# hku-mars/FAST_LIO

Measured on NVIDIA H100. Metric: scans/sec (30k-pt scan, 1M-pt map iEKF), higher is better.
Workload: dtype f32 geometry / f64 filter

## Files before the change

fast_lio_b200/csrc/filter.cu:

```cuda
#include <dlfcn.h>

#include <algorithm>
#include <chrono>
#include <cstdlib>

#include <cub/device/device_select.cuh>

#include "filter.h"
#include "gj.cuh"

namespace fl {

constexpr int PSTRIDE = 96;
constexpr size_t P2P_MAIL_BYTES = sizeof(unsigned long long) * 2 * 2 * P2P_MAX_RANKS * PSTRIDE;
constexpr int SEARCH_THREADS = 256;
constexpr int SEARCH_C_THREADS = 256;
constexpr int RESID_THREADS = 256;
constexpr int MAX_LOGS = 16;

__device__ __forceinline__ void pdl_wait() { asm volatile("griddepcontrol.wait;" ::: "memory"); }
__device__ __forceinline__ void pdl_launch() { asm volatile("griddepcontrol.launch_dependents;" ::: "memory"); }

__device__ __forceinline__ int tri12(int a, int b) { return a * 12 - (a * (a - 1)) / 2 + (b - a); }

// ... 960 lines not shown

__global__ void k_flags_clear(unsigned char* __restrict__ flag_add, unsigned char* __restrict__ flag_no, const int* __restrict__ n, int n_max) {
    const int q = blockIdx.x * blockDim.x + threadIdx.x;
    if (q < n_max && q >= *n) { flag_add[q] = 0; flag_no[q] = 0; }
}

struct NcclUniqueId { char internal[128]; };
struct NcclApi {
    void* lib = nullptr;
    int (*GetUniqueId)(NcclUniqueId*) = nullptr;
    int (*CommInitRank)(void**, int, NcclUniqueId, int) = nullptr;
    int (*AllReduce)(const void*, void*, size_t, int, int, void*, cudaStream_t) = nullptr;
    int (*CommDestroy)(void*) = nullptr;
    const char* (*GetErrorString)(int) = nullptr;
};
static NcclApi* load_nccl() {
    static NcclApi api;
    if (api.lib) return &api;
    const char* names[] = {"libnccl.so.2", "libnccl.so"};
    for (const char* nm : names) { api.lib = dlopen(nm, RTLD_NOW | RTLD_GLOBAL); if (api.lib) break; }
    if (!api.lib) { set_last_error("NCCL: cannot dlopen libnccl.so.2: %s", dlerror()); return nullptr; }
    api.GetUniqueId = (int (*)(NcclUniqueId*))dlsym(api.lib, "ncclGetUniqueId");
    api.CommInitRank = (int (*)(void**, int, NcclUniqueId, int))dlsym(api.lib, "ncclCommInitRank");
    api.AllReduce = (int (*)(const void*, void*, size_t, int, int, void*, cudaStream_t))dlsym(api.lib, "ncclAllReduce");
    api.CommDestroy = (int (*)(void*))dlsym(api.lib, "ncclCommDestroy");
    api.GetErrorString = (const char* (*)(int))dlsym(api.lib, "ncclGetErrorString");
    if (!api.GetUniqueId || !api.CommInitRank || !api.AllReduce || !api.CommDestroy) {
        set_last_error("NCCL: missing symbols in libnccl");
        api.lib = nullptr;
        return nullptr;
    }
    return &api;
}
int nccl_unique_id(void* out128) {
    NcclApi* api = load_nccl();
    if (!api) return FL_ERR_NCCL;
    NcclUniqueId id;
    int rc = api->GetUniqueId(&id);
    if (rc != 0) { set_last_error("ncclGetUniqueId failed: %d", rc); return FL_ERR_NCCL; }
    memcpy(out128, &id, 128);
    return FL_OK;
}

Filter::Filter(Map* map, int max_points) : map_(map), max_points_(max_points) {
    memset(&scan_, 0, sizeof(scan_));
    for (int i = 0; i < NDOF; i++) limit_[i] = 0.001;
}
Filter::~Filter() {
    cudaSetDevice(map_->device());
    if (comm_ && nccl_) nccl_->CommDestroy(comm_);
    for (int r = 0; r < P2P_MAX_RANKS; r++) if (peer_ptr_[r]) cudaIpcCloseMemHandle(peer_ptr_[r]);
    mailbox_.release(); p2p_.release();
    body_.release(); nearest_.release(); nearest_cnt_.release(); selected_.release(); normvec_.release(); plane_.release(); srange_.release();
    partials_.release(); red_.release(); ctl_.release(); ctl0_.release(); logs_.release(); pub_.release();
    mi_world_.release(); mi_flag_add_.release(); mi_flag_no_.release(); mi_list_add_.release(); mi_list_no_.release(); mi_tmp_.release(); mi_counts_.release();
    d_bind_.release();
    if (h_ctl_) cudaFreeHost(h_ctl_);
    if (ev0_) cudaEventDestroy(ev0_);
    if (ev1_) cudaEventDestroy(ev1_);
}

int Filter::init() {
    FL_CUDA(cudaSetDevice(map_->device()));
    if (const char* e = getenv("FASTLIO_B200_NO_PDL")) pdl_ = !(e[0] == '1');
    if (const char* e = getenv("FASTLIO_B200_NO_MIRROR")) mirror_ = !(e[0] == '1');
    if (const char* e = getenv("FASTLIO_B200_SEARCH")) search_mode_ = atoi(e) ? 1 : 0;
    FL_CHECK(ctl_.reserve(sizeof(FilterCtl)));
    FL_CHECK(ctl0_.reserve(sizeof(FilterCtl)));
    FL_CHECK(red_.reserve(sizeof(double) * PSTRIDE));
    FL_CHECK(logs_.reserve(sizeof(PassLog) * MAX_LOGS));
    FL_CHECK(pub_.reserve(512));
    FL_CUDA(cudaMemsetAsync(pub_.ptr, 0, 512, stream()));
    FL_CUDA(cudaMallocHost(&h_ctl_, sizeof(FilterCtl)));
    memset(h_ctl_, 0, sizeof(FilterCtl));
    FL_CUDA(cudaMemsetAsync(ctl_.ptr, 0, sizeof(FilterCtl), stream()));
    FL_CUDA(cudaMemsetAsync(ctl0_.ptr, 0, sizeof(FilterCtl), stream()));
    FL_CUDA(cudaMemsetAsync(logs_.ptr, 0, sizeof(PassLog) * MAX_LOGS, stream()));
    int dev = map_->device(), occ = 0;
    FL_CUDA(cudaDeviceGetAttribute(&sms_, cudaDevAttrMultiProcessorCount, dev));
    if (const char* e = getenv("FASTLIO_B200_SEARCH_OCC")) search_occ_ = atoi(e);
    if (search_occ_ == 6) FL_CUDA(cudaOccupancyMaxActiveBlocksPerMultiprocessor(&occ, k_search<6>, SEARCH_THREADS, 0));
    else if (search_occ_ == 5) FL_CUDA(cudaOccupancyMaxActiveBlocksPerMultiprocessor(&occ, k_search<5>, SEARCH_THREADS, 0));
    else FL_CUDA(cudaOccupancyMaxActiveBlocksPerMultiprocessor(&occ, k_search<4>, SEARCH_THREADS, 0));
    search_grid_max_ = sms_ * std::max(1, occ);
    if (const char* e = getenv("FASTLIO_B200_LEGACY")) fused_ = !(e[0] == '1');
    FL_CUDA(cudaOccupancyMaxActiveBlocksPerMultiprocessor(&occ, k_update<false, 1>, UPD_THREADS, 0));
    upd_capacity_[0][0] = sms_ * std::max(1, occ);
    FL_CUDA(cudaOccupancyMaxActiveBlocksPerMultiprocessor(&occ, k_update<true, 1>, UPD_THREADS, 0));
    upd_capacity_[1][0] = sms_ * std::max(1, occ);
    FL_CUDA(cudaOccupancyMaxActiveBlocksPerMultiprocessor(&occ, k_update<false, 2>, 2 * UPD_THREADS, 0));
    upd_capacity_[0][1] = sms_ * occ;
    FL_CUDA(cudaOccupancyMaxActiveBlocksPerMultiprocessor(&occ, k_update<true, 2>, 2 * UPD_THREADS, 0));
    upd_capacity_[1][1] = sms_ * occ;
    FL_CUDA(cudaOccupancyMaxActiveBlocksPerMultiprocessor(&occ, k_update_n<false, 1>, UPD_THREADS, 0));
    upd_n_capacity_[0][0] = std::min(upd_capacity_[0][0], sms_ * std::max(1, occ));
    FL_CUDA(cudaOccupancyMaxActiveBlocksPerMultiprocessor(&occ, k_update_n<true, 1>, UPD_THREADS, 0));
    upd_n_capacity_[1][0] = std::min(upd_capacity_[1][0], sms_ * std::max(1, occ));
    FL_CUDA(cudaOccupancyMaxActiveBlocksPerMultiprocessor(&occ, k_update_n<false, 2>, 2 * UPD_THREADS, 0));
    upd_n_capacity_[0][1] = std::min(upd_capacity_[0][1], sms_ * occ);
    FL_CUDA(cudaOccupancyMaxActiveBlocksPerMultiprocessor(&occ, k_update_n<true, 2>, 2 * UPD_THREADS, 0));
    upd_n_capacity_[1][1] = std::min(upd_capacity_[1][1], sms_ * occ);
    FL_CHECK(d_bind_.reserve(2 * sizeof(int)));
    FL_CUDA(cudaMemsetAsync(d_bind_.ptr, 0, 2 * sizeof(int), stream()));
    FL_CHECK(partials_.reserve(sizeof(double) * PSTRIDE * (size_t)std::max(upd_capacity_[0][0], upd_capacity_[1][0])));
    max_resid_grid_ = sms_;
    FL_CHECK(partials_.reserve(sizeof(double) * PSTRIDE * (size_t)max_resid_grid_));
    FL_CHECK(reserve(std::max(1, max_points_)));
    return FL_OK;
}

int Filter::reserve(int nq) {
    FL_CHECK(body_.reserve(sizeof(float4) * (size_t)nq));
    FL_CHECK(nearest_.reserve(sizeof(float4) * KNN_K * (size_t)nq));
    { const size_t had = nearest_cnt_.bytes; FL_CHECK(nearest_cnt_.reserve(sizeof(int) * (size_t)nq)); if (nearest_cnt_.bytes != had) FL_CUDA(cudaMemsetAsync(nearest_cnt_.ptr, 0, nearest_cnt_.bytes, stream())); }
    FL_CHECK(selected_.reserve((size_t)nq));
    FL_CHECK(normvec_.reserve(sizeof(float4) * (size_t)nq));
    scan_.nearest = nearest_.as<float4>();
    scan_.nearest_cnt = nearest_cnt_.as<int>();
    scan_.selected = selected_.as<unsigned char>();
    scan_.normvec = normvec_.as<float4>();
    FL_CHECK(plane_.reserve(sizeof(float4) * (size_t)nq));
    scan_.plane = plane_.as<float4>();
    FL_CHECK(srange_.reserve(sizeof(double) * (size_t)nq));
    scan_.srange = srange_.as<double>();
    FL_CHECK(mi_world_.reserve(sizeof(float4) * (size_t)nq));
    FL_CHECK(mi_flag_add_.reserve((size_t)nq));
    FL_CHECK(mi_flag_no_.reserve((size_t)nq));
    FL_CHECK(mi_list_add_.reserve(sizeof(float4) * (size_t)nq));
    FL_CHECK(mi_list_no_.reserve(sizeof(float4) * (size_t)nq));
    FL_CHECK(mi_counts_.reserve(sizeof(int) * 2));
    size_t tmp = 0;
    FL_CUDA(cub::DeviceSelect::Flagged(nullptr, tmp, (const float4*)nullptr, (const unsigned char*)nullptr, (float4*)nullptr, (int*)nullptr, nq));
    FL_CHECK(mi_tmp_.reserve(tmp));
    return FL_OK;
}

int Filter::set_params(int max_iter, const double* limit23, int extrinsic_est_en) {
    if (max_iter < 1 || max_iter + 1 > MAX_LOGS) { set_last_error("set_params: max_iter must be in [1, %d]", MAX_LOGS - 1); return FL_ERR_ARG; }
    max_iter_ = max_iter;
    if (limit23) for (int i = 0; i < NDOF; i++) limit_[i] = limit23[i];
    extrinsic_est_ = extrinsic_est_en ? 1 : 0;
    return FL_OK;
}

int Filter::set_scan_device(const float4* d_body, int nq) {
    FL_CHECK(bind_scan(d_body, nq));
    if (stream_bound_) FL_CUDA(cudaMemsetAsync(d_bind_.as<int>() + 1, 0, sizeof(int), stream()));
    return FL_OK;
}
int Filter::bind_scan(const float4* d_body, int nq) {
    if (nq < 0) { set_last_error("scan: nq < 0"); return FL_ERR_ARG; }
    FL_CUDA(cudaSetDevice(map_->device()));
    FL_CHECK(reserve(std::max(1, nq)));
    scan_.body = d_body;
    scan_.Q = nq;
    if (!shard_set_) { scan_.q_begin = 0; scan_.q_end = nq; }
    dev_count_ = false;
    return FL_OK;
// ... 87 lines not shown
        if (nranks_ > 1 && !p2p_on_) {
            for (int pass = 0; pass <= max_iter_; pass++) {
                FL_CHECK(launch_update(1, 1, 0));
                int rc = nccl_->AllReduce(red_.ptr, red_.ptr, NRED,  8,  0, comm_, st);
                if (rc != 0) { set_last_error("ncclAllReduce failed: %d", rc); return FL_ERR_NCCL; }
                FL_CHECK(launch_update(1, 3, 0));
                launches_ += 2;
            }
        } else {
            FL_CHECK(launch_update(max_iter_ + 1, nranks_ > 1 ? 2 : 0, 0));
            launches_ = 1;
        }
        FL_CUDA(cudaGetLastError());
        return FL_OK;
    }
    for (int pass = 0; pass <= max_iter_; pass++) {
        FL_CHECK(launch_search_only());
        FL_CHECK(launch_residual_only());
        launches_ += 2;
        if (nranks_ > 1 && !p2p_on_) {
            cudaStream_t st = stream();
            int rc = nccl_->AllReduce(red_.ptr, red_.ptr, NRED,  8,  0, comm_, st);
            if (rc != 0) { set_last_error("ncclAllReduce failed: %d", rc); return FL_ERR_NCCL; }
            FilterCtl* c = ctl_.as<FilterCtl>(); double* rg = red_.as<double>(); PassLog* lg = logs_.as<PassLog>();
            if (extrinsic_est_) { if (solver_) k_solve_only<true, 1><<<1, RESID_THREADS, 0, st>>>(c, rg, scan_, lg); else k_solve_only<true, 0><<<1, RESID_THREADS, 0, st>>>(c, rg, scan_, lg); }
            else { if (solver_) k_solve_only<false, 1><<<1, RESID_THREADS, 0, st>>>(c, rg, scan_, lg); else k_solve_only<false, 0><<<1, RESID_THREADS, 0, st>>>(c, rg, scan_, lg); }
            launches_++;
        }
    }
    FL_CUDA(cudaGetLastError());
    return FL_OK;
}

UpdArgs Filter::upd_args(int max_passes, int mode, int search_only) {
    UpdArgs a;
    a.m = map_->view();
    if (search_mode_ == 0) a.m.dir.cap = 0;
    a.sc = scan_; a.ctl = ctl_.as<FilterCtl>(); a.partials = partials_.as<double>(); a.red_g = red_.as<double>();
    a.logs = logs_.as<PassLog>(); a.p2p = p2p_.as<P2PState>();
    a.mode = mode; a.max_passes = max_passes; a.search_only = search_only;
    a.pub = pub_.as<unsigned long long>(); a.nonce = ++launch_nonce_;
    { const char* e = getenv("FASTLIO_B200_DBG"); a.dbg = e ? atoi(e) : 0; }
    a.pose_from_search = 0;
    return a;
}

int Filter::launch_update(int max_passes, int mode, int search_only, cudaStream_t st) {
    FL_CUDA(cudaSetDevice(map_->device()));
    const int nq = scan_.q_end - scan_.q_begin;
    const UpdArgs a = upd_args(max_passes, mode, search_only);
    const int cap = upd_capacity_[extrinsic_est_ ? 1 : 0][0];
    int workers = mode == 3 ? 0 : std::min(cap - 1, (nq + UPD_THREADS - 1) / UPD_THREADS);
    if (workers < 0) workers = 0;
    FL_CUDA(launch_upd(workers, pdl_, a, upd_pair(nq), st));
    return FL_OK;
}

int Filter::upd_pair(int nq) const {
    if (const char* e = getenv("FASTLIO_B200_PAIR")) if (e[0] == '1') return 1;
    const int tiles = (nq + UPD_THREADS - 1) / UPD_THREADS;
    return tiles >= 1 && tiles <= upd_capacity_[extrinsic_est_ ? 1 : 0][1] - 1 ? 2 : 1;
}
cudaError_t Filter::launch_upd(int workers, bool pdl, const UpdArgs& a, int pair, cudaStream_t st) {
    const int block = pair * UPD_THREADS;
    if (extrinsic_est_) return pair == 2 ? launch_pdl(k_update<true, 2>, workers + 1, block, st, pdl, a)
                                         : launch_pdl(k_update<true, 1>, workers + 1, block, st, pdl, a);
    return pair == 2 ? launch_pdl(k_update<false, 2>, workers + 1, block, st, pdl, a)
                     : launch_pdl(k_update<false, 1>, workers + 1, block, st, pdl, a);
}

int Filter::launch_search_only() {
    FL_CUDA(cudaSetDevice(map_->device()));
    const int nq = scan_.q_end - scan_.q_begin;
    if (fused()) return launch_update(1, 0, 1);
    if (search_mode_ == 1) {
        const int cgrid = std::max(1, (nq + SEARCH_C_THREADS - 1) / SEARCH_C_THREADS);
        FL_CUDA(launch_pdl(k_search_c, cgrid, SEARCH_C_THREADS, stream(), pdl_, map_->view(), scan_, (const FilterCtl*)ctl_.as<FilterCtl>()));
        return FL_OK;
    }
    const int sgrid = std::max(1, std::min(search_grid_max_, (nq * 32 + SEARCH_THREADS - 1) / SEARCH_THREADS));
    const FilterCtl* cc = ctl_.as<FilterCtl>();
    if (search_occ_ == 6) FL_CUDA(launch_pdl(k_search<6>, sgrid, SEARCH_THREADS, stream(), pdl_, map_->view(), scan_, cc));
    else if (search_occ_ == 5) FL_CUDA(launch_pdl(k_search<5>, sgrid, SEARCH_THREADS, stream(), pdl_, map_->view(), scan_, cc));
    else FL_CUDA(launch_pdl(k_search<4>, sgrid, SEARCH_THREADS, stream(), pdl_, map_->view(), scan_, cc));
    return FL_OK;
}
int Filter::launch_residual_only() {
    FL_CUDA(cudaSetDevice(map_->device()));
    const int nq = scan_.q_end - scan_.q_begin;
    resid_grid_ = std::min(max_resid_grid_ - 1, (nq + RESID_THREADS - 1) / RESID_THREADS) + 1;
    const int mode = nranks_ > 1 ? (p2p_on_ ? 2 : 1) : 0;
    P2PState* p2p = p2p_.as<P2PState>();
    FilterCtl* c = ctl_.as<FilterCtl>(); double* pp = partials_.as<double>(); double* rg = red_.as<double>(); PassLog* lg = logs_.as<PassLog>();
    cudaStream_t st = stream();
    if (extrinsic_est_) {
        if (solver_) FL_CUDA(launch_pdl(k_residual<true, 1>, resid_grid_, RESID_THREADS, st, pdl_, scan_, c, pp, rg, mode, lg, p2p));
        else FL_CUDA(launch_pdl(k_residual<true, 0>, resid_grid_, RESID_THREADS, st, pdl_, scan_, c, pp, rg, mode, lg, p2p));
    } else {
        if (solver_) FL_CUDA(launch_pdl(k_residual<false, 1>, resid_grid_, RESID_THREADS, st, pdl_, scan_, c, pp, rg, mode, lg, p2p));
        else FL_CUDA(launch_pdl(k_residual<false, 0>, resid_grid_, RESID_THREADS, st, pdl_, scan_, c, pp, rg, mode, lg, p2p));
    }
    FL_CUDA(cudaGetLastError());
    return FL_OK;
}
int Filter::sync() {
    FL_CUDA(cudaSetDevice(map_->device()));
    FL_CUDA(cudaStreamSynchronize(stream()));
    return FL_OK;
}

int Filter::download_state(double* x26, double* P, int* n_pass) {
    FL_CUDA(cudaSetDevice(map_->device()));
    FL_CUDA(cudaStreamSynchronize(stream()));
    if (!(mirror_ && h_ctl_->done)) {
        FL_CUDA(cudaMemcpyAsync(h_ctl_, ctl_.ptr, offsetof(FilterCtl, P_prop), cudaMemcpyDeviceToHost, stream()));
        FL_CUDA(cudaStreamSynchronize(stream()));
    }
// ... 383 lines not shown
```

fast_lio_b200/csrc/filter.h:

```cpp
#pragma once
#include "lie.cuh"
#include "map.h"

namespace fl {

struct PassLog {
    int searched, valid, effct, converged;
    double res_sum;
    double HtH[144];
    double Hth[12];
    double x_after[XLEN];
};

struct FilterCtl {
    int iter;
    int t;
    int converge;
    int done;
    int n_pass;
    int max_iter;
    int extrinsic_est;
    int error;
    int ticket;
    int gen;
// ... 54 lines not shown
    int launch_residual_only();
    int download_state(double* x26, double* P, int* n_pass);
    int sync();
    int update_on_stream(const float* d_body, int nq, double* d_x26, double* d_P, double R, int* d_status2, cudaStream_t st);
    int get_nearest_on_stream(float* d_pts, int* d_cnt, int nq, cudaStream_t st);
    int get_selected_on_stream(unsigned char* d_out, int nq, cudaStream_t st);
    int update_scan_on_stream(const float4* d_body, const int* d_n, int n_max, double* d_x26, double* d_P, double R, int* d_status2, cudaStream_t st);
    int capacity() const;

    int map_incremental(double filter_size_map_min, int ekf_inited, int* n_to_add, int* n_no_downsample, int* added);
    int map_incremental_on_stream(double filter_size_map_min, int ekf_inited, int* d_out4, cudaStream_t st);
    int get_nearest(float* out_pts, int* out_cnt, int nq);
    int complete_neighbours();
    int get_selected(unsigned char* out, int nq);
    int get_pass_logs(PassLog* out, int cap, int* n);
    int comm_init(int nranks, int rank, const void* nccl_unique_id_128);
    int set_shard(int q_begin, int q_end);
    int p2p_local_handle(void* out64);
    int p2p_connect(int nranks, int rank, const void* handles64);
    int p2p_barrier();

    void set_fused(bool on) { fused_ = on; }
    bool fused() const { return fused_ && solver_ == 1; }
    int gpu_launches() const { return launches_; }
    const long long* host_ns() const { return host_ns_; }
    const float4* nearest_device() const { return scan_.nearest; }
    const ScanView& scan() const { return scan_; }
    cudaStream_t stream() const { return map_->stream(); }
    Map* map() const { return map_; }
    const FilterCtl* ctl_device() const { return ctl_.as<FilterCtl>(); }

private:
    int reserve(int nq);
    int update_any(const float* body_xyzi, const float4* d_body, int nq, double* x26, double* P, double R, double* solve_time_s);
    Map* map_;
    int max_points_;
    int max_iter_ = 4;
    double limit_[NDOF];
    int extrinsic_est_ = 0;
    int solver_ = 1;
    bool mirror_ = true;
    bool pdl_ = true;
    int search_occ_ = 5;
    int search_mode_ = 1;
    ScanView scan_;
    DeviceBuffer srange_;
    DeviceBuffer body_, nearest_, nearest_cnt_, selected_, normvec_, plane_, partials_, red_, ctl_, ctl0_, logs_;
    DeviceBuffer mi_world_, mi_flag_add_, mi_flag_no_, mi_list_add_, mi_list_no_, mi_tmp_, mi_counts_;
    FilterCtl* h_ctl_ = nullptr;
    cudaEvent_t ev0_ = nullptr, ev1_ = nullptr;
    int sms_ = 0, search_grid_max_ = 0, max_resid_grid_ = 0, resid_grid_ = 1;
    bool fused_ = true;
    DeviceBuffer pub_;
    unsigned launch_nonce_ = 0;
    int upd_capacity_[2][2] = {{0, 0}, {0, 0}};
    int launch_update(int max_passes, int mode, int search_only) { return launch_update(max_passes, mode, search_only, stream()); }
    int launch_update(int max_passes, int mode, int search_only, cudaStream_t st);
    int upd_pair(int nq) const;
    cudaError_t launch_upd(int workers, bool pdl, const UpdArgs& a, int pair) { return launch_upd(workers, pdl, a, pair, stream()); }
    cudaError_t launch_upd(int workers, bool pdl, const UpdArgs& a, int pair, cudaStream_t st);
    int device_form_scope(const char* what, bool update) const;
    UpdArgs upd_args(int max_passes, int mode, int search_only);
    int bind_scan(const float4* d_body, int nq);
    bool dev_count_ = false;
    int q_max_ = 0;
    const float4* scan_body_ = nullptr;
    bool stream_bound_ = false;
    DeviceBuffer d_bind_;
    int upd_n_capacity_[2][2] = {{0, 0}, {0, 0}};
    int read_binding();
    int launches_ = 0;
    long long host_ns_[4] = {0, 0, 0, 0};
    bool shard_set_ = false;
    bool neighbours_complete_ = true;
    NcclApi* nccl_ = nullptr;
    void* comm_ = nullptr;
    int nranks_ = 1, rank_ = 0;
    DeviceBuffer mailbox_, p2p_;
    void* peer_ptr_[P2P_MAX_RANKS] = {nullptr};
    bool p2p_on_ = false;
};

}
```

fast_lio_b200/csrc/update.cuh:

```cuda
#pragma once

namespace fl {

constexpr int UPD_THREADS = 256;
constexpr int UPD_WARPS = UPD_THREADS / 32;

struct UpdArgs {
    MapView m;
    ScanView sc;
    FilterCtl* ctl;
    double* partials;
    double* red_g;
    PassLog* logs;
    P2PState* p2p;
    unsigned long long* pub;
    unsigned nonce;
    int mode;
    int max_passes;
    int search_only;
    int dbg;
    int pose_from_search;
};

struct SolverSm {
    double Pp[NDOF * NDOF];
    double Pt[NDOF * NDOF];
    double W1[NDOF * NDOF];
    double Y[12 * NDOF];
    double Wm[12 * 13];
    double HTH[144];
    double wred[UPD_WARPS][PSTRIDE];
    double red[PSTRIDE];
    double x[XLEN], xprop[XLEN], xnew[XLEN];
    double dx[NDOF], dxn[NDOF], dxu[NDOF], limit[NDOF];
    double J[2][9], M2[4];
    double Bprop[6];
    double R;
    int iter, t, converge, done, n_pass, max_iter, error;
    int effct, ok, finish, searched, late;
    int row_k[12];
};
template <bool EXTR> struct WorkerSm {
    static constexpr int STAGE = 32 * RowStage<EXTR>::RS + 96;
    double stage[UPD_WARPS][STAGE];
    double wred[UPD_WARPS][PSTRIDE];
    WalkPool walks;
    unsigned pose_bits[28];
    unsigned flags;
    int abort;
};

__device__ __forceinline__ int ld_acquire(const int* p) {
    int v;
    asm volatile("ld.acquire.gpu.global.s32 %0, [%1];" : "=r"(v) : "l"(p) : "memory");
    return v;
}
__device__ __forceinline__ void st_release(int* p, int v) { asm volatile("st.release.gpu.global.s32 [%0], %1;" ::"l"(p), "r"(v) : "memory"); }
constexpr long long SPIN_LIMIT = 3000000000ll;

constexpr int PUB_WORDS = 29;
__device__ __forceinline__ unsigned pub_tag(unsigned nonce, int pass) { return (nonce << 8) | (unsigned)(pass & 0xff); }
__device__ __forceinline__ void pub_store(unsigned long long* p, unsigned tag, unsigned payload) {
    asm volatile("st.relaxed.gpu.global.u64 [%0], %1;" ::"l"(p), "l"(((unsigned long long)tag << 32) | payload) : "memory");
}
__device__ __forceinline__ unsigned long long pub_load(const unsigned long long* p) {
    unsigned long long v;
    asm volatile("ld.relaxed.gpu.global.u64 %0, [%1];" : "=l"(v) : "l"(p) : "memory");
    return v;
}
__device__ __forceinline__ void pub_publish(unsigned long long* pub, unsigned tag, const double* x, int converge, int done, int lane) {
    if (lane < 28) {
        const unsigned long long bits = (unsigned long long)__double_as_longlong(x[lane >> 1]);
        pub_store(pub + lane, tag, (lane & 1) ? (unsigned)(bits >> 32) : (unsigned)bits);
    } else if (lane == 28) {
        pub_store(pub + 28, tag, (converge ? 1u : 0u) | (done ? 2u : 0u));
    }
}


__device__ __forceinline__ void cell_scan_chunks(const MapView& m, int start, int cnt, int c0, int c1, float qx, float qy, float qz, TBest& kb) {
    const int4* list = reinterpret_cast<const int4*>(m.dir.lists + start);
    int4 ia = make_int4(0, 0, 0, 0), ib = make_int4(0, 0, 0, 0);
    if (c0 < c1) {
        ia = __ldg(&list[2 * c0]);
        if (cnt - 8 * c0 > 4) ib = __ldg(&list[2 * c0 + 1]);
    }
#pragma unroll 1
    for (int c = c0; c < c1; c++) {
        const int n8 = cnt - 8 * c;
        float4 p0, p1, p2, p3, p4, p5, p6, p7;
        p1 = p2 = p3 = p4 = p5 = p6 = p7 = make_float4(0.f, 0.f, 0.f, 0.f);
        p0 = __ldg(&m.pts[ia.x]);
        if (n8 > 1) p1 = __ldg(&m.pts[ia.y]);
        if (n8 > 2) p2 = __ldg(&m.pts[ia.z]);
        if (n8 > 3) p3 = __ldg(&m.pts[ia.w]);
        if (n8 > 4) p4 = __ldg(&m.pts[ib.x]);
        if (n8 > 5) p5 = __ldg(&m.pts[ib.y]);
        if (n8 > 6) p6 = __ldg(&m.pts[ib.z]);
        if (n8 > 7) p7 = __ldg(&m.pts[ib.w]);
        int4 na = ia, nb = ib;
        if (c + 1 < c1) {
            na = __ldg(&list[2 * c + 2]);
            if (n8 > 12) nb = __ldg(&list[2 * c + 3]);
        }
        cell_consider(p0, ia.x, qx, qy, qz, kb);
        cell_consider(p1, ia.y, qx, qy, qz, kb);
        cell_consider(p2, ia.z, qx, qy, qz, kb);
        cell_consider(p3, ia.w, qx, qy, qz, kb);
        cell_consider(p4, ib.x, qx, qy, qz, kb);
        cell_consider(p5, ib.y, qx, qy, qz, kb);
        cell_consider(p6, ib.z, qx, qy, qz, kb);
        cell_consider(p7, ib.w, qx, qy, qz, kb);
        ia = na; ib = nb;
    }
}

struct PairXch {
    float d[KNN_K][32];
    int idx[KNN_K][32];
};

__device__ __forceinline__ void pair_merge(const PairXch& X, int lane, TBest& kb) {
// ... 178 lines not shown
#pragma unroll 1
            for (int i = 0; i < 9; i++) S.J[warp][i] = J.m[i];
            const D3 seg = mul33v(J, l);
            S.dx[idx] = l.x; S.dx[idx + 1] = l.y; S.dx[idx + 2] = l.z;
            S.dxn[idx] = seg.x; S.dxn[idx + 1] = seg.y; S.dxn[idx + 2] = seg.z;
        } else if (warp == 2) {
            double d0, d1;
            S2_boxminus_B(ld3(S.x + X_GRAV), ld3(S.xprop + X_GRAV), S.Bprop, d0, d1);
            S2_congruence_B(ld3(S.x + X_GRAV), ld3(S.xprop + X_GRAV), S.Bprop, d0, d1, S.M2);
            S.dx[21] = d0; S.dx[22] = d1;
            S.dxn[21] = S.M2[0] * d0 + S.M2[1] * d1;
            S.dxn[22] = S.M2[2] * d0 + S.M2[3] * d1;
        }
    }
    if (warp == 3 && lane < 15) {
        const int b = lane / 3, c = lane % 3;
        const int dof = b == 0 ? 0 : 9 + 3 * (b - 1);
        const int xo = b == 0 ? X_POS : (b == 1 ? X_OFFT : (b == 2 ? X_VEL : (b == 3 ? X_BG : X_BA)));
        const double d = S.x[xo + c] - S.xprop[xo + c];
        S.dx[dof + c] = d; S.dxn[dof + c] = d;
    }
    sol_sync();
#pragma unroll 1
    for (int e = tid; e < n * n; e += UPD_THREADS) {
        const int i = e / n, j = e - i * n;
        const double* row = &S.Pp[i * n];
        double v;
        if (j >= 3 && j < 9) {
            const int b = j >= 6, base = 3 + 3 * b, r = j - base;
            v = S.J[b][3 * r] * row[base] + S.J[b][3 * r + 1] * row[base + 1] + S.J[b][3 * r + 2] * row[base + 2];
        } else if (j >= 21) {
            const int r = j - 21;
            v = S.M2[2 * r] * row[21] + S.M2[2 * r + 1] * row[22];
        } else v = row[j];
        S.W1[e] = v;
    }
    sol_sync();
#pragma unroll 1
    for (int e = tid; e < n * n; e += UPD_THREADS) {
        const int i = e / n, j = e - i * n;
        double v;
        if (i >= 3 && i < 9) {
            const int b = i >= 6, base = 3 + 3 * b, r = i - base;
            v = S.J[b][3 * r] * S.W1[base * n + j] + S.J[b][3 * r + 1] * S.W1[(base + 1) * n + j] + S.J[b][3 * r + 2] * S.W1[(base + 2) * n + j];
        } else if (i >= 21) {
            const int r = i - 21;
            v = S.M2[2 * r] * S.W1[21 * n + j] + S.M2[2 * r + 1] * S.W1[22 * n + j];
        } else v = S.W1[e];
        S.Pt[e] = v;
    }
    sol_sync();
}

__device__ void sol_reduce(SolverSm& S, const double* __restrict__ partials, int nwork) {
    const int tid = threadIdx.x, lane = tid & 31, warp = tid >> 5;
    double a0 = 0.0, a1 = 0.0, a2 = 0.0;
    for (int b = warp; b < nwork; b += 8 * UPD_WARPS) {
        double v[8][3];
#pragma unroll
        for (int k = 0; k < 8; k++) {
            const int bb = b + k * UPD_WARPS;
            const double* row = partials + (size_t)bb * PSTRIDE;
            v[k][0] = v[k][1] = v[k][2] = 0.0;
            if (bb < nwork) { v[k][0] = __ldcg(&row[lane]); v[k][1] = __ldcg(&row[lane + 32]); v[k][2] = __ldcg(&row[lane + 64]); }
        }
#pragma unroll
        for (int k = 0; k < 8; k++) { a0 += v[k][0]; a1 += v[k][1]; a2 += v[k][2]; }
    }
    S.wred[warp][lane] = a0; S.wred[warp][lane + 32] = a1; S.wred[warp][lane + 64] = a2;
    sol_sync();
    if (tid < PSTRIDE) {
        double v = 0.0;
#pragma unroll
        for (int w = 0; w < UPD_WARPS; w++) v += S.wred[w][tid];
        S.red[tid] = v;
        if (tid < 78) {
            int a = 0, rem = tid;
            while (rem >= 12 - a) { rem -= 12 - a; a++; }
            const int b = a + rem;
            S.HTH[a * 12 + b] = v; S.HTH[b * 12 + a] = v;
        }
    }
    sol_sync();
}
__device__ void sol_expand(SolverSm& S) {
    const int tid = threadIdx.x;
    if (tid < 144) { const int a = tid / 12, b = tid - a * 12; S.HTH[tid] = S.red[a <= b ? tri12(a, b) : tri12(b, a)]; }
    sol_sync();
}

__device__ void sol_exchange(SolverSm& S, P2PState* p2p) {
    const int nr = p2p->nranks, me = p2p->rank;
    const unsigned long long epoch = p2p->epoch + 1;
    const unsigned long long tag = (epoch & 0xffffffffull) << 32;
    const int par = (int)(epoch & 1ull);
    for (int idx = threadIdx.x; idx < nr * PSTRIDE; idx += UPD_THREADS) {
        const int r = idx / PSTRIDE, o = idx - r * PSTRIDE;
        const unsigned long long bits = (unsigned long long)__double_as_longlong(S.red[o]);
        unsigned long long* dst = reinterpret_cast<unsigned long long*>(p2p->peer_mail[r]) + (((size_t)par * nr + me) * PSTRIDE + o) * 2;
        asm volatile("st.volatile.global.u64 [%0], %1;" ::"l"(dst), "l"(tag | (bits & 0xffffffffull)) : "memory");
        asm volatile("st.volatile.global.u64 [%0], %1;" ::"l"(dst + 1), "l"(tag | (bits >> 32)) : "memory");
    }
    sol_sync();
    if (threadIdx.x < PSTRIDE) {
        const unsigned long long* mail = reinterpret_cast<const unsigned long long*>(p2p->peer_mail[me]) + (size_t)par * nr * PSTRIDE * 2;
        double v = 0.0;
        bool late = false;
        for (int r = 0; r < nr && !late; r++) {
            const unsigned long long* src = mail + ((size_t)r * PSTRIDE + threadIdx.x) * 2;
            unsigned long long lo = 0, hi = 0;
            const long long t0 = clock64();
            while (true) {
                asm volatile("ld.volatile.global.u64 %0, [%1];" : "=l"(lo) : "l"(src) : "memory");
                asm volatile("ld.volatile.global.u64 %0, [%1];" : "=l"(hi) : "l"(src + 1) : "memory");
                if ((lo & 0xffffffff00000000ull) == tag && (hi & 0xffffffff00000000ull) == tag) break;
                if (clock64() - t0 > SPIN_LIMIT) { late = true; break; }
            }
            v += __longlong_as_double((long long)((hi << 32) | (lo & 0xffffffffull)));
        }
        S.red[threadIdx.x] = v;
// ... 122 lines not shown
        }
        asm volatile("bar.sync 1, 128;" ::: "memory");
#pragma unroll 1
        for (int e = t4; e < n * n; e += 128) {
            const int i = e / n, j = e - i * n;
            double v = 0.0;
#pragma unroll
            for (int a = 0; a < NE; a++) v = fma(S.Pt[i * n + a] * Rinv, S.Y[a * n + j], v);
            S.W1[e] = S.Pt[e] - v;
        }
    }
    sol_sync();
    if (tid < XLEN) { ctl->x[tid] = S.xnew[tid]; if (lg) lg->x_after[tid] = S.xnew[tid]; }
    if (tid == 32) { ctl->t = S.t; ctl->converge = S.converge; ctl->iter = S.iter + 1; ctl->n_pass = S.n_pass + 1; ctl->done = finish; }
    if (!finish) {
#pragma unroll 1
        for (int e = tid; e < n * n; e += UPD_THREADS) ctl->P[e] = S.Pt[e];
    } else {
#pragma unroll 1
        for (int e = tid; e < n * n; e += UPD_THREADS) {
            const int i = e / n, j = e - i * n;
            double v;
            if (i >= 3 && i < 9) {
                const int b = i >= 6, base = 3 + 3 * b, r = i - base;
                v = S.J[b][3 * r] * S.W1[base * n + j] + S.J[b][3 * r + 1] * S.W1[(base + 1) * n + j] + S.J[b][3 * r + 2] * S.W1[(base + 2) * n + j];
            } else if (i >= 21) {
                const int r = i - 21;
                v = S.M2[2 * r] * S.W1[21 * n + j] + S.M2[2 * r + 1] * S.W1[22 * n + j];
            } else v = S.W1[e];
            S.Pt[e] = v;
        }
        sol_sync();
#pragma unroll 1
        for (int e = tid; e < n * n; e += UPD_THREADS) {
            const int i = e / n, j = e - i * n;
            const double* row = &S.Pt[i * n];
            double v;
            if (j >= 3 && j < 9) {
                const int b = j >= 6, base = 3 + 3 * b, r = j - base;
                v = S.J[b][3 * r] * row[base] + S.J[b][3 * r + 1] * row[base + 1] + S.J[b][3 * r + 2] * row[base + 2];
            } else if (j >= 21) {
                const int r = j - 21;
                v = S.M2[2 * r] * row[21] + S.M2[2 * r + 1] * row[22];
            } else v = row[j];
            ctl->P[e] = v;
        }
    }
    sol_sync();
    if (tid < XLEN) S.x[tid] = S.xnew[tid];
    if (tid == 32) { S.iter++; S.n_pass++; S.done = finish; }
    sol_sync();
}

template <bool EXTR, int PAIR>
__device__ __forceinline__ void update_body(const UpdArgs& a, const int q1) {
    static_assert(PAIR == 1 || PAIR == 2, "one or two threads per point");
    static_assert(sizeof(PairXch) <= sizeof(double) * WorkerSm<EXTR>::STAGE, "the partner's list fits the owner warp's stage slice");
    __shared__ __align__(16) unsigned char smem_raw[sizeof(SolverSm) > sizeof(WorkerSm<EXTR>) ? sizeof(SolverSm) : sizeof(WorkerSm<EXTR>)];
    FilterCtl* ctl = a.ctl;
    const int tid = threadIdx.x, lane = tid & 31, warp = tid >> 5;
    const int nwork = (int)gridDim.x - 1;
    pdl_wait();
    pdl_launch();
    if (blockIdx.x > 0) {
        WorkerSm<EXTR>& Wk = *reinterpret_cast<WorkerSm<EXTR>*>(smem_raw);
        const int wb = (int)blockIdx.x - 1;
        if (tid == 0) { Wk.abort = 0; Wk.walks.n[0] = Wk.walks.n[1] = 0; }
        __syncthreads();
        int walk_phase = 0;
        for (int p = 0; p < a.max_passes; p++) {
            PoseS s;
            bool searched;
            if (p == 0) {
                if (__ldcg(&ctl->done) && !a.search_only) return;
                searched = __ldcg(&ctl->converge) != 0 || a.search_only;
                s = load_pose(a.pose_from_search ? ctl->x_search : ctl->x);
            } else {
                const unsigned tag = pub_tag(a.nonce, p);
                if (tid == 0) {
                    const long long t0 = clock64();
                    while ((unsigned)(pub_load(a.pub + 28) >> 32) != tag) {
                        if (clock64() - t0 > SPIN_LIMIT) { Wk.abort = 1; atomicExch(&ctl->error, 3); break; }
                        __nanosleep((a.dbg & 1) ? 2000 : 100);
                    }
                }
                __syncthreads();
                if (Wk.abort) return;
                if (tid < PUB_WORDS) {
                    unsigned long long w = pub_load(a.pub + tid);
                    const long long t0 = clock64();
                    while ((unsigned)(w >> 32) != tag && clock64() - t0 < SPIN_LIMIT) w = pub_load(a.pub + tid);
                    if (tid < 28) Wk.pose_bits[tid] = (unsigned)w; else Wk.flags = (unsigned)w;
                }
                __syncthreads();
                if (Wk.flags & 2u) return;
                searched = (Wk.flags & 1u) != 0;
                double x14[14];
#pragma unroll
                for (int i = 0; i < 14; i++) x14[i] = __longlong_as_double((long long)(((unsigned long long)Wk.pose_bits[2 * i + 1] << 32) | Wk.pose_bits[2 * i]));
                s.pos = d3(x14[X_POS], x14[X_POS + 1], x14[X_POS + 2]);
                s.rot.x = x14[X_ROT]; s.rot.y = x14[X_ROT + 1]; s.rot.z = x14[X_ROT + 2]; s.rot.w = x14[X_ROT + 3];
                s.offR.x = x14[X_OFFR]; s.offR.y = x14[X_OFFR + 1]; s.offR.z = x14[X_OFFR + 2]; s.offR.w = x14[X_OFFR + 3];
                s.offT = d3(x14[X_OFFT], x14[X_OFFT + 1], x14[X_OFFT + 2]);
            }
            double acc[3] = {0.0, 0.0, 0.0};
            const bool owner = PAIR == 1 || tid < UPD_THREADS;
            double* stage = Wk.stage[warp & (UPD_WARPS - 1)];
            const int q0 = a.sc.q_begin;
            for (int tile = q0 + wb * UPD_THREADS; tile < q1; tile += nwork * UPD_THREADS) {
                const int q = tile + (tid & (UPD_THREADS - 1));
                double h[12]; double z = 0.0; float ar = 0.f;
                bool contrib = false;
                if (owner || searched)
                    contrib = measure_fused<EXTR, PAIR>(a.m, a.sc, q, q < q1, s, searched, a.search_only != 0, Wk.walks, walk_phase, stage, h, z, ar);
                if (owner && !a.search_only) warp_accumulate<EXTR>(contrib, h, z, ar, acc, lane, stage);
            }
            if (a.search_only) return;
            if (owner) {
#pragma unroll
                for (int j = 0; j < 3; j++) Wk.wred[warp][lane + 32 * j] = acc[j];
            }
            __syncthreads();
            if (tid < PSTRIDE) {
                double v = 0.0;
#pragma unroll
                for (int w = 0; w < UPD_WARPS; w++) v += Wk.wred[w][tid];
                __stcg(&a.partials[(size_t)wb * PSTRIDE + tid], v);
            }
            __syncthreads();
            if (tid == 0) asm volatile("red.release.gpu.global.add.s32 [%0], 1;" ::"l"(&ctl->ticket) : "memory");
            if (a.mode == 1) return;
        }
        return;
    }
    if (a.search_only) return;
    if (tid >= UPD_THREADS) return;
    SolverSm& S = *reinterpret_cast<SolverSm*>(smem_raw);
    sol_load(S, ctl);
    int p = 0;
    for (; p < a.max_passes && !S.done; p++) {
        if (tid == 0) ctl->prof[0] = clock64();
        if (S.converge && tid < XLEN) ctl->x_search[tid] = S.x[tid];
        if (a.mode != 1) sol_prepare(S);
        if (tid == 0) ctl->prof[8] = clock64();
        if (a.mode != 3) {
            if (tid == 0) {
                const long long t0 = clock64();
                while (ld_acquire(&ctl->ticket) < nwork * (p + 1)) {
                    if (clock64() - t0 > SPIN_LIMIT) { S.late = 2; break; }
                }
            }
            sol_sync();
            if (tid == 0) ctl->prof[9] = clock64();
            sol_reduce(S, a.partials, nwork);
            if (a.mode == 1) {
                if (tid < NRED) a.red_g[tid] = S.red[tid];
                if (tid == 0) ctl->ticket = 0;
                return;
            }
        } else {
            if (tid < PSTRIDE) S.red[tid] = tid < NRED ? a.red_g[tid] : 0.0;
            sol_sync();
            sol_expand(S);
        }
        if (a.mode == 2) { sol_exchange(S, a.p2p); sol_expand(S); }
        if (tid == 0) ctl->prof[1] = clock64();
        sol_pass<EXTR>(S, ctl, a.logs, a.pub, pub_tag(a.nonce, p + 1));
        if (tid == 0) ctl->prof[7] = clock64();
    }
    if (tid == 0) { ctl->error = S.error | ctl->error; ctl->ticket = 0; }
    sol_sync();
    mirror_copy(ctl, UPD_THREADS);
}

template <bool EXTR, int PAIR>
__global__ void __launch_bounds__(UPD_THREADS * PAIR, 3 - PAIR) k_update(UpdArgs a) {
    update_body<EXTR, PAIR>(a, a.sc.q_end);
}

template <bool EXTR, int PAIR>
__global__ void __launch_bounds__(UPD_THREADS * PAIR, 3 - PAIR) k_update_n(UpdArgs a, const int* __restrict__ n) {
    update_body<EXTR, PAIR>(a, min(*n, a.sc.q_end));
}

}
```

Baseline: 11660.

## Replace worker ticket counter with self-tagged partial rows in update kernel

Adds an alternative update-kernel path for small worker counts in mode 0. Each worker writes its partial sums as tagged 64-bit pairs (the sequence and pass tag sit next to each half of the double), and the solver block polls those rows directly instead of waiting on a global atomic ticket and then reading the partials. The worker pose wait is also spread across a warp with nanosleep backoff. This is meant to remove the atomic round trip and the serialized ticket spin before the reduction. In exchange it doubles the partial-row traffic, adds a persistent sequence counter in the pub buffer, and relies on relaxed vector stores being observed atomically.

```diff
diff --git a/fast_lio_b200/csrc/filter.cu b/fast_lio_b200/csrc/filter.cu
--- a/fast_lio_b200/csrc/filter.cu
+++ b/fast_lio_b200/csrc/filter.cu
@@ -1036,7 +1036,7 @@
     for (int r = 0; r < P2P_MAX_RANKS; r++) if (peer_ptr_[r]) cudaIpcCloseMemHandle(peer_ptr_[r]);
     mailbox_.release(); p2p_.release();
     body_.release(); nearest_.release(); nearest_cnt_.release(); selected_.release(); normvec_.release(); plane_.release(); srange_.release();
-    partials_.release(); red_.release(); ctl_.release(); ctl0_.release(); logs_.release(); pub_.release();
+    partials_.release(); red_.release(); ctl_.release(); ctl0_.release(); logs_.release(); pub_.release(); rows_.release();
     mi_world_.release(); mi_flag_add_.release(); mi_flag_no_.release(); mi_list_add_.release(); mi_list_no_.release(); mi_tmp_.release(); mi_counts_.release();
     d_bind_.release();
     if (h_ctl_) cudaFreeHost(h_ctl_);
@@ -1088,6 +1088,11 @@
     FL_CUDA(cudaMemsetAsync(d_bind_.ptr, 0, 2 * sizeof(int), stream()));
     FL_CHECK(partials_.reserve(sizeof(double) * PSTRIDE * (size_t)std::max(upd_capacity_[0][0], upd_capacity_[1][0])));
     max_resid_grid_ = sms_;
+    {
+        const size_t rows = sizeof(unsigned long long) * 2 * PSTRIDE * TAGGED_WORKERS;
+        FL_CHECK(rows_.reserve(rows));
+        FL_CUDA(cudaMemsetAsync(rows_.ptr, 0, rows, stream()));
+    }
     FL_CHECK(partials_.reserve(sizeof(double) * PSTRIDE * (size_t)max_resid_grid_));
     FL_CHECK(reserve(std::max(1, max_points_)));
     return FL_OK;
@@ -1281,7 +1286,7 @@
     const int cap = upd_capacity_[extrinsic_est_ ? 1 : 0][0];
     int workers = mode == 3 ? 0 : std::min(cap - 1, (nq + UPD_THREADS - 1) / UPD_THREADS);
     if (workers < 0) workers = 0;
-    FL_CUDA(launch_upd(workers, pdl_, a, upd_pair(nq), st));
+    FL_CUDA(launch_upd(workers, pdl_, a, upd_pair(nq), st, mode == 0 && workers <= TAGGED_WORKERS));
     return FL_OK;
 }
 
@@ -1290,8 +1295,16 @@
     const int tiles = (nq + UPD_THREADS - 1) / UPD_THREADS;
     return tiles >= 1 && tiles <= upd_capacity_[extrinsic_est_ ? 1 : 0][1] - 1 ? 2 : 1;
 }
-cudaError_t Filter::launch_upd(int workers, bool pdl, const UpdArgs& a, int pair, cudaStream_t st) {
+cudaError_t Filter::launch_upd(int workers, bool pdl, const UpdArgs& a0, int pair, cudaStream_t st, bool r1) {
     const int block = pair * UPD_THREADS;
+    UpdArgs a = a0;
+    if (r1) {
+        a.partials = rows_.as<double>();
+        if (extrinsic_est_) return pair == 2 ? launch_pdl(k_update_1r<true, 2>, workers + 1, block, st, pdl, a)
+                                             : launch_pdl(k_update_1r<true, 1>, workers + 1, block, st, pdl, a);
+        return pair == 2 ? launch_pdl(k_update_1r<false, 2>, workers + 1, block, st, pdl, a)
+                         : launch_pdl(k_update_1r<false, 1>, workers + 1, block, st, pdl, a);
+    }
     if (extrinsic_est_) return pair == 2 ? launch_pdl(k_update<true, 2>, workers + 1, block, st, pdl, a)
                                          : launch_pdl(k_update<true, 1>, workers + 1, block, st, pdl, a);
     return pair == 2 ? launch_pdl(k_update<false, 2>, workers + 1, block, st, pdl, a)
diff --git a/fast_lio_b200/csrc/filter.h b/fast_lio_b200/csrc/filter.h
--- a/fast_lio_b200/csrc/filter.h
+++ b/fast_lio_b200/csrc/filter.h
@@ -130,13 +130,14 @@
     int sms_ = 0, search_grid_max_ = 0, max_resid_grid_ = 0, resid_grid_ = 1;
     bool fused_ = true;
     DeviceBuffer pub_;
+    DeviceBuffer rows_;
     unsigned launch_nonce_ = 0;
     int upd_capacity_[2][2] = {{0, 0}, {0, 0}};
     int launch_update(int max_passes, int mode, int search_only) { return launch_update(max_passes, mode, search_only, stream()); }
     int launch_update(int max_passes, int mode, int search_only, cudaStream_t st);
     int upd_pair(int nq) const;
     cudaError_t launch_upd(int workers, bool pdl, const UpdArgs& a, int pair) { return launch_upd(workers, pdl, a, pair, stream()); }
-    cudaError_t launch_upd(int workers, bool pdl, const UpdArgs& a, int pair, cudaStream_t st);
+    cudaError_t launch_upd(int workers, bool pdl, const UpdArgs& a, int pair, cudaStream_t st, bool r1 = false);
     int device_form_scope(const char* what, bool update) const;
     UpdArgs upd_args(int max_passes, int mode, int search_only);
     int bind_scan(const float4* d_body, int nq);
diff --git a/fast_lio_b200/csrc/update.cuh b/fast_lio_b200/csrc/update.cuh
--- a/fast_lio_b200/csrc/update.cuh
+++ b/fast_lio_b200/csrc/update.cuh
@@ -68,6 +68,21 @@
     asm volatile("ld.relaxed.gpu.global.u64 %0, [%1];" : "=l"(v) : "l"(p) : "memory");
     return v;
 }
+constexpr int PUB_SEQ = 31;
+constexpr int TAGGED_WORKERS = 4 * UPD_WARPS;
+__device__ __forceinline__ unsigned row_tag(unsigned seq, int pass) { return pub_tag(seq, pass + 1); }
+__device__ __forceinline__ void row_store(unsigned long long* p, unsigned tag, double v) {
+    const unsigned long long bits = (unsigned long long)__double_as_longlong(v), t = (unsigned long long)tag << 32;
+    asm volatile("st.relaxed.gpu.global.v2.u64 [%0], {%1, %2};" ::"l"(p), "l"(t | (bits & 0xffffffffull)), "l"(t | (bits >> 32)) : "memory");
+}
+__device__ __forceinline__ ulonglong2 row_load(const unsigned long long* p) {
+    ulonglong2 v;
+    asm volatile("ld.relaxed.gpu.global.v2.u64 {%0, %1}, [%2];" : "=l"(v.x), "=l"(v.y) : "l"(p) : "memory");
+    return v;
+}
+__device__ __forceinline__ bool row_current(ulonglong2 v, unsigned tag) { return (unsigned)(v.x >> 32) == tag && (unsigned)(v.y >> 32) == tag; }
+__device__ __forceinline__ double row_value(ulonglong2 v) { return __longlong_as_double((long long)((v.y << 32) | (v.x & 0xffffffffull))); }
+
 __device__ __forceinline__ void pub_publish(unsigned long long* pub, unsigned tag, const double* x, int converge, int done, int lane) {
     if (lane < 28) {
         const unsigned long long bits = (unsigned long long)__double_as_longlong(x[lane >> 1]);
@@ -352,9 +367,46 @@
     sol_sync();
 }
 
-__device__ void sol_reduce(SolverSm& S, const double* __restrict__ partials, int nwork) {
+template <bool R1 = false>
+__device__ void sol_reduce(SolverSm& S, const double* __restrict__ partials, int nwork, unsigned tag = 0u) {
     const int tid = threadIdx.x, lane = tid & 31, warp = tid >> 5;
     double a0 = 0.0, a1 = 0.0, a2 = 0.0;
+    if constexpr (R1) {
+        const unsigned long long* rows = reinterpret_cast<const unsigned long long*>(partials);
+        const long long t0 = clock64();
+        bool late = false;
+        for (int b = warp; b < nwork; b += 4 * UPD_WARPS) {
+            ulonglong2 v[4][3];
+#pragma unroll
+            for (int k = 0; k < 4; k++) {
+                const int bb = b + k * UPD_WARPS;
+#pragma unroll
+                for (int c = 0; c < 3; c++) v[k][c] = bb < nwork ? row_load(rows + ((size_t)bb * PSTRIDE + lane + 32 * c) * 2) : make_ulonglong2(0ull, 0ull);
+            }
+            while (!late) {
+                bool stale = false;
+#pragma unroll
+                for (int k = 0; k < 4; k++)
+#pragma unroll
+                    for (int c = 0; c < 3; c++) stale |= b + k * UPD_WARPS < nwork && !row_current(v[k][c], tag);
+                if (!stale) break;
+                if (clock64() - t0 > SPIN_LIMIT) { late = true; break; }
+#pragma unroll
+                for (int k = 0; k < 4; k++) {
+                    const int bb = b + k * UPD_WARPS;
+#pragma unroll
+                    for (int c = 0; c < 3; c++)
+                        if (bb < nwork && !row_current(v[k][c], tag)) v[k][c] = row_load(rows + ((size_t)bb * PSTRIDE + lane + 32 * c) * 2);
+                }
+            }
+#pragma unroll
+            for (int k = 0; k < 4; k++) {
+                const bool in = b + k * UPD_WARPS < nwork;
+                a0 += in ? row_value(v[k][0]) : 0.0; a1 += in ? row_value(v[k][1]) : 0.0; a2 += in ? row_value(v[k][2]) : 0.0;
+            }
+        }
+        if (late) S.late = 2;
+    } else {
     for (int b = warp; b < nwork; b += 8 * UPD_WARPS) {
         double v[8][3];
 #pragma unroll
@@ -366,6 +418,7 @@
         }
 #pragma unroll
         for (int k = 0; k < 8; k++) { a0 += v[k][0]; a1 += v[k][1]; a2 += v[k][2]; }
+    }
     }
     S.wred[warp][lane] = a0; S.wred[warp][lane + 32] = a1; S.wred[warp][lane + 64] = a2;
     sol_sync();
@@ -594,7 +647,7 @@
     sol_sync();
 }
 
-template <bool EXTR, int PAIR>
+template <bool EXTR, int PAIR, bool R1 = false>
 __device__ __forceinline__ void update_body(const UpdArgs& a, const int q1) {
     static_assert(PAIR == 1 || PAIR == 2, "one or two threads per point");
     static_assert(sizeof(PairXch) <= sizeof(double) * WorkerSm<EXTR>::STAGE, "the partner's list fits the owner warp's stage slice");
@@ -604,6 +657,8 @@
     const int nwork = (int)gridDim.x - 1;
     pdl_wait();
     pdl_launch();
+    unsigned seq = 0u;
+    if constexpr (R1) seq = (unsigned)pub_load(a.pub + PUB_SEQ);
     if (blockIdx.x > 0) {
         WorkerSm<EXTR>& Wk = *reinterpret_cast<WorkerSm<EXTR>*>(smem_raw);
         const int wb = (int)blockIdx.x - 1;
@@ -619,6 +674,24 @@
                 s = load_pose(a.pose_from_search ? ctl->x_search : ctl->x);
             } else {
                 const unsigned tag = pub_tag(a.nonce, p);
+                if constexpr (R1) {
+                    if (warp == 0) {
+                        unsigned long long w = 0ull;
+                        const long long t0 = clock64();
+                        while (true) {
+                            if (lane < PUB_WORDS) w = pub_load(a.pub + lane);
+                            if (__all_sync(FULL, lane >= PUB_WORDS || (unsigned)(w >> 32) == tag)) break;
+                            if (__shfl_sync(FULL, clock64() - t0 > SPIN_LIMIT, 0)) {
+                                if (lane == 0) { Wk.abort = 1; atomicExch(&ctl->error, 3); }
+                                break;
+                            }
+                            __nanosleep((a.dbg & 1) ? 2000 : 100);
+                        }
+                        if (lane < 28) Wk.pose_bits[lane] = (unsigned)w; else if (lane == 28) Wk.flags = (unsigned)w;
+                    }
+                    __syncthreads();
+                    if (Wk.abort) return;
+                } else {
                 if (tid == 0) {
                     const long long t0 = clock64();
                     while ((unsigned)(pub_load(a.pub + 28) >> 32) != tag) {
@@ -635,6 +708,7 @@
                     if (tid < 28) Wk.pose_bits[tid] = (unsigned)w; else Wk.flags = (unsigned)w;
                 }
                 __syncthreads();
+                }
                 if (Wk.flags & 2u) return;
                 searched = (Wk.flags & 1u) != 0;
                 double x14[14];
@@ -667,10 +741,13 @@
                 double v = 0.0;
 #pragma unroll
                 for (int w = 0; w < UPD_WARPS; w++) v += Wk.wred[w][tid];
-                __stcg(&a.partials[(size_t)wb * PSTRIDE + tid], v);
-            }
+                if constexpr (R1) row_store(reinterpret_cast<unsigned long long*>(a.partials) + ((size_t)wb * PSTRIDE + tid) * 2, row_tag(seq, p), v);
+                else __stcg(&a.partials[(size_t)wb * PSTRIDE + tid], v);
+            }
+            if constexpr (!R1) {
             __syncthreads();
             if (tid == 0) asm volatile("red.release.gpu.global.add.s32 [%0], 1;" ::"l"(&ctl->ticket) : "memory");
+            }
             if (a.mode == 1) return;
         }
         return;
@@ -686,6 +763,9 @@
         if (a.mode != 1) sol_prepare(S);
         if (tid == 0) ctl->prof[8] = clock64();
         if (a.mode != 3) {
+            if constexpr (R1) {
+                sol_reduce<true>(S, a.partials, nwork, row_tag(seq, p));
+            } else {
             if (tid == 0) {
                 const long long t0 = clock64();
                 while (ld_acquire(&ctl->ticket) < nwork * (p + 1)) {
@@ -695,6 +775,7 @@
             sol_sync();
             if (tid == 0) ctl->prof[9] = clock64();
             sol_reduce(S, a.partials, nwork);
+            }
             if (a.mode == 1) {
                 if (tid < NRED) a.red_g[tid] = S.red[tid];
                 if (tid == 0) ctl->ticket = 0;
@@ -711,6 +792,9 @@
         if (tid == 0) ctl->prof[7] = clock64();
     }
     if (tid == 0) { ctl->error = S.error | ctl->error; ctl->ticket = 0; }
+    if constexpr (R1) {
+        if (tid == 0 && p > 0) pub_store(a.pub + PUB_SEQ, 0u, seq + 1u);
+    }
     sol_sync();
     mirror_copy(ctl, UPD_THREADS);
 }
@@ -721,6 +805,11 @@
 }
 
 template <bool EXTR, int PAIR>
+__global__ void __launch_bounds__(UPD_THREADS * PAIR, 3 - PAIR) k_update_1r(UpdArgs a) {
+    update_body<EXTR, PAIR, true>(a, a.sc.q_end);
+}
+
+template <bool EXTR, int PAIR>
 __global__ void __launch_bounds__(UPD_THREADS * PAIR, 3 - PAIR) k_update_n(UpdArgs a, const int* __restrict__ n) {
     update_body<EXTR, PAIR>(a, min(*n, a.sc.q_end));
 }
```

After: 11660 (median of 6 runs). No clear change (-0.0%).
